# luk036/ellalgo-rs

Hardware: AMD Instinct MI355X
Metric: ellipsoid updates/sec at n=16384; achieved HBM GB/s vs peak (higher is better)
Workload: dtype f64

## Files before the change

ellalgo-rs_amd/capi.py:

```python
from __future__ import annotations

import ctypes as C
import os

from . import build as _build

SUCCESS, NOSOLN, NOEFFECT, UNKNOWN = 0, 1, 2, 3
CUT_BIAS, CUT_CENTRAL, CUT_Q = 0, 1, 2
SPACE_ELL, SPACE_ELL_STABLE = 0, 1
E_NORCCL = -6
SHARD_EQUAL_BLOCKS, SHARD_SYMMETRIC = 0, 1
NCCL_ID_BYTES = 128
E_INVALID, E_HIP, E_NODEVICE, E_NOMEM, E_STATE = -1, -2, -3, -4, -5
NKERNEL_CLASSES = 14
(OPT_AUTO_DEFER, OPT_SYMV, OPT_SYMV_MIN_N, OPT_APPLY_LOWER, OPT_APPLY_KERNEL, OPT_FUSE_DOTS, OPT_STABLE_SOLVE,
 OPT_STABLE_FACTOR, OPT_PAD, OPT_LP_GRID, OPT_LP_WIDE, OPT_BATCH_THREADS, OPT_RESIDENT, OPT_OVERLAP,
 OPT_LOOKAHEAD, OPT_QUEUE_DEPTH, OPT_RESIDENT_FAULT, OPT_RESIDENT_ABANDONED, OPT_STABLE_MIRRORED, OPT_STAGE_DIRECT) = range(1, 21)
KERNEL_CLASS_NAMES = ("gemv", "scalar", "rank1", "stable_fwd", "stable_bwd", "stable_factor", "fused", "apply",
                      "apply_gemv", "symv", "symv_reduce", "lp_scan", "lp_final", "resident")

EXPORTS = [
    "ellhip_create", "ellhip_create_shard", "ellhip_clone", "ellhip_destroy", "ellhip_update", "ellhip_tsq",
    "ellhip_get_xc", "ellhip_set_xc", "ellhip_kappa", "ellhip_ndim", "ellhip_get_mq",
    "ellhip_set_no_defer_trick", "ellhip_set_use_parallel_cut", "ellhip_set_defer_depth", "ellhip_defer_depth", "ellhip_flush", "ellhip_queue_primed", "ellhip_set_shard_symmetric", "ellhip_calc", "ellhip_update_begin",
    "ellhip_update_end", "ellhip_gt_dev", "ellhip_set_gt_dev", "ellhip_prime", "ellhip_cut", "ellhip_commit",
    "ellhip_queue_upload", "ellhip_queue_run", "ellhip_queue_run_fused", "ellhip_queue_begin", "ellhip_queue_end",
    "ellhip_queue_prime", "ellhip_queue_cut", "ellhip_queue_commit", "ellhip_queue_results", "ellhip_set_stream",
    "ellhip_synchronize", "ellhip_profile_enable", "ellhip_profile_read", "ellhip_device_count",
    "ellhip_last_error", "ellhip_version",
    "ellhip_set_option", "ellhip_get_option", "ellhip_set_default_option", "ellhip_default_option",
    "ellhip_lowpass_create", "ellhip_lowpass_destroy", "ellhip_lowpass_assess_feas", "ellhip_lowpass_assess_optim",
    "ellhip_lowpass_state", "ellhip_lowpass_rows_visited", "ellhip_lowpass_get_spectrum", "ellhip_lowpass_optim", "ellhip_lowpass_feas",
# ... 240 lines not shown
```

ellalgo-rs_amd/csrc/ell_kernels.hpp:

```cpp
#pragma once

#include <hip/hip_runtime.h>

#include "ellcalc_device.hpp"

namespace ellhip {

struct CutParams {
    int kind;
    int has_b1;
    double b0;
    double b1;
};

struct DevState {
    double kappa;
    double tsq;
    double omega;
    double ratio;
    double rho_over_omega;
    double scale;
    int status;
    int apply;
    int halted;
// ... 1068 lines not shown
    __shared__ double sgr[SYMV_H][SMM_NV2 + 1];
    __shared__ int s_t;
    if (st->halted) return;
    Q -= row0 * ld;
    for (;;) {
        __syncthreads();
        if (threadIdx.x == 0) {
            const unsigned t = atomicAdd(queue, 1u);
            s_t = t < (unsigned)ntiles ? (int)t : -1;
        }
        __syncthreads();
        const int t = s_t;
        if (t < 0) return;
        symm_tile2<NT, SEG>(Q, ld, n, row0, (long long)tiles[t].I, (long long)tiles[t].J, gT, lv, rowpart, colpart, rowpart_stride,
                            colpart_stride, sh, sgr);
    }
}

constexpr int PUB_WGS = 16;
__global__ __launch_bounds__(256) void k_publish(const DevState* __restrict__ st, const double* __restrict__ xc, long long n,
                                                 LiveMirror* __restrict__ m, double* __restrict__ h_xc,
                                                 unsigned long long seq, unsigned* __restrict__ arrived) {
    __shared__ int last;
    const long long n2 = n / 2;
    for (long long i = (long long)blockIdx.x * 256 + threadIdx.x; i < n2; i += (long long)gridDim.x * 256)
        *reinterpret_cast<double2_t*>(h_xc + 2 * i) = *reinterpret_cast<const double2_t*>(xc + 2 * i);
    if ((n & 1) && blockIdx.x == 0 && threadIdx.x == 0) h_xc[n - 1] = xc[n - 1];
    __threadfence_system();
    __syncthreads();
    if (threadIdx.x == 0) {
// ... 530 lines not shown
```

ellalgo-rs_amd/csrc/ellhip_capi.hip:

```cpp
#include "../../include/ellhip.h"

#include <hip/hip_runtime.h>

#include <cstddef>
#include <cstdio>
#include <cstdlib>
#include <algorithm>
#include <atomic>
#include <cstring>
#include <memory>
#include <mutex>
#include <new>
#include <string>
#include <vector>

#include "ell_kernels.hpp"
#include "ellstable_kernels.hpp"
#include "resident_kernels.hpp"
#include "group_kernels.hpp"

using namespace ellhip;

namespace {

// ... 24 lines not shown
    hipEvent_t a, b;
    int cls;
};

struct Defaults {
    int auto_defer = 1;
    int symv = 1;
    long long symv_min_n = 5120;
    int apply_lower = 1;
    int apply_kernel = -1;
    int fuse_dots = 1;
    int resident = 1;
    int overlap = 1;
    int lookahead = 32;
    int queue_depth = 48;
    int stable_solve = 3;
    int stable_factor = 2;
    int pad = -1;
    int lp_grid = 0;
    int lp_wide = -1;
    int batch_threads = 0;
    int stage_direct = 1;
};
Defaults g_defaults;

enum : int { CLS_GEMV = 0, CLS_SCALAR = 1, CLS_RANK1 = 2, CLS_ST_FWD = 3, CLS_ST_BWD = 4, CLS_ST_FACTOR = 5, CLS_FUSED = 6, CLS_APPLY = 7, CLS_APPLY_GEMV = 8, CLS_SYMV = 9, CLS_SYMV_REDUCE = 10, CLS_LP_SCAN = 11, CLS_LP_FINAL = 12, CLS_RESIDENT = 13 };

struct Shape {
    int rw = 0, unr = 0, nt = 0;
};
// ... 28 lines not shown
    int st_since_enter = 0;
    bool st_prev_persist = true;
    bool st_prev_helped = true;
    double* d_partial = nullptr;
    double* d_pend = nullptr;
    double* d_cpend = nullptr;
    double* d_rowpart = nullptr;
    double* d_colpart = nullptr;
    int overlap = 1;
    double* d_rowpart2 = nullptr;
    double* d_colpart2 = nullptr;
    int part_set = 0;
    hipStream_t symv_stream = nullptr;
    int lookahead = 32;
    int queue_depth = 48;
    double* d_rowpart_m = nullptr;
    double* d_colpart_m = nullptr;
    double* d_gT = nullptr;
    SymmTile* d_symm_tiles = nullptr;
    unsigned* d_symm_queue = nullptr;
    int symm_ntiles = 0, symm_wgs = 0;
    double* d_grpY = nullptr;
    double* d_gpart = nullptr;
    double* d_cpart = nullptr;
    double* d_gsums = nullptr;
    GroupOut* d_gout = nullptr;
    int (*grp_exchange)(void* ctx, double* buf, long long count, hipStream_t stream) = nullptr;
    void* grp_exchange_ctx = nullptr;
    hipEvent_t ev_symv = nullptr;
    hipEvent_t ev_side_go = nullptr;
// ... 139 lines not shown
        s->sh_fused = {4, 4, 0};
    } else {
        s->sh_gemv = {4, 4, 1};
        s->sh_rank1 = {2, 8, 1};
        s->sh_fused = {2, 8, 1};
    }
    s->sh_apply = {4, 1, s->sh_fused.nt};
    s->symv = g_defaults.symv;
    s->symv_min_n = g_defaults.symv_min_n;
    s->apply_lower = g_defaults.apply_lower;
    s->apply_kernel = g_defaults.apply_kernel;
    s->fuse_dots = g_defaults.fuse_dots;
    s->overlap = g_defaults.overlap;
    s->lookahead = g_defaults.lookahead;
    s->queue_depth = g_defaults.queue_depth;
    s->resident = g_defaults.resident;
    s->stable_solve = g_defaults.stable_solve;
    s->stable_factor = g_defaults.stable_factor;
}

template <int VEC, bool NT, bool R1, bool GV, bool SCALE>
int launch_sweep_t(ellhip_space* s, const Shape& sh, const double* gt_r1, const double* gvec, double* gv_out) {
    const long long nr = s->nrows;
    const unsigned grid = (unsigned)((nr + sh.rw - 1) / sh.rw);
    double* out = gv_out ? gv_out + s->row0 : nullptr;
#define SWEEP_CASE(RW, UNR)                                                                                  \
    if (sh.rw == RW && sh.unr == UNR) {                                                                      \
        hipLaunchKernelGGL((k_sweep<RW, UNR, VEC, NT, R1, GV, SCALE>), dim3(grid), dim3(256), 0, s->stream,  \
                           (const double*)s->d_Q, s->d_Q, s->ld, s->n, nr, s->row0, gt_r1, gvec, out, s->d_st, \
                           s->dir);                                                                          \
// ... 72 lines not shown
#define APPLY_CASE(RW, UNR)                                                                                   \
    if (sh.rw == RW && sh.unr == UNR) {                                                                       \
        hipLaunchKernelGGL((k_sweep_apply<RW, UNR, VEC, NT, GV, LOWER>), dim3(grid), dim3(256), 0, s->stream, \
                           (const double*)s->d_Q, s->d_Q, s->ld, s->n, nr, s->row0, (const double*)s->d_pend, \
                           (const double*)s->d_cpend, gvec, out, s->d_st, dir);                               \
        return 0;                                                                                             \
    }
    APPLY_CASE(1, 2) APPLY_CASE(1, 4) APPLY_CASE(2, 1) APPLY_CASE(2, 2) APPLY_CASE(2, 4) APPLY_CASE(4, 1) APPLY_CASE(4, 2)
#undef APPLY_CASE
    return fail(ELLHIP_E_INVALID, "unsupported ELLHIP_APPLY_RW/UNR shape (supported: 1x2 1x4 2x1 2x2 2x4 4x1 4x2)");
}

bool symv_ok(const ellhip_space* s);

int side_join(ellhip_space* s);
int flush_pending(ellhip_space* s, const double* gvec, double* gv_out) {
    {
        int jrc = side_join(s);
        if (jrc) return jrc;
        ProfScope ps(s, gvec ? CLS_APPLY_GEMV : CLS_APPLY);
        const bool even = (s->n % 2) == 0;
        const bool nt = even && s->sh_apply.nt;
        int rc;
        if (!gvec && s->apply_lower && symv_ok(s)) {
            const unsigned grid = (unsigned)((s->nrows + APL_TR - 1) / APL_TR);
#define APL_GO(NPV, NTV)                                                                                        \
    hipLaunchKernelGGL((k_apply_lower<NPV, NTV>), dim3(grid), dim3(256), 0, s->stream, s->d_Q, s->ld, s->n, s->nrows, \
                       s->row0, (const double*)s->d_pend, (const double*)s->d_cpend, (const DevState*)s->d_st)
            const bool deep = s->npend > s->defer;
            const int apply_kernel = deep ? 2 : (s->apply_kernel < 0 ? (s->defer == 24 ? 2 : 1) : s->apply_kernel);
// ... 22 lines not shown
            rc = 0;
            s->upper_stale = true;
        } else if (s->defer != 8) {
            return fail(ELLHIP_E_STATE, "defer depth 16 / 24 needs the lower-triangle schedule");
        } else if (gvec)
            rc = !even ? launch_apply_t<1, false, true>(s, gvec, gv_out)
                       : (nt ? launch_apply_t<2, true, true>(s, gvec, gv_out) : launch_apply_t<2, false, true>(s, gvec, gv_out));
        else
            rc = !even ? launch_apply_t<1, false, false>(s, nullptr, nullptr)
                       : (nt ? launch_apply_t<2, true, false>(s, nullptr, nullptr)
                             : launch_apply_t<2, false, false>(s, nullptr, nullptr));
        if (rc) return rc;
        HIPCHK(hipGetLastError());
        s->dir ^= 1;
    }
    hipLaunchKernelGGL(k_pend_reset, dim3(64), dim3(256), 0, s->stream, s->d_pend, s->d_cpend,
                       (long long)(s->npend > s->defer ? MAXPEND : s->defer) * s->n, s->d_st);
    HIPCHK(hipGetLastError());
    s->npend = 0;
    return 0;
}

int launch_mirror_if_needed(ellhip_space* s) {
    if (!s->needs_mirror) return 0;
    const unsigned t = (unsigned)((s->n + 31) / 32);
    hipLaunchKernelGGL(k_mirror_lower, dim3(t, t), dim3(256), 0, s->stream, s->d_Q, s->ld, s->n, s->d_st);
    HIPCHK(hipGetLastError());
    return 0;
}

constexpr int ST_MIRROR_PERIOD = 256;
int stable_mirror_enter(ellhip_space* s) {
    const unsigned t = (unsigned)((s->n + 63) / 64);
    hipLaunchKernelGGL(k_st_mirror_enter, dim3(t, t), dim3(256), 0, s->stream, s->d_Q, s->ld, s->n, (const DevState*)s->d_st,
                       s->d_rbuf);
// ... 967 lines not shown
                       (long long)colpart_elems(s), (const DevState*)s->d_st, (const SymmTile*)s->d_symm_tiles, 0, s->d_symm_queue)
        if (wide && nt) {
            ELLHIP_SYMM_WARM(k_symm_mfma_q<true, SYMV_SEG>);
            ELLHIP_SYMM_WARM(k_symm_mfma_q2<true, SYMV_SEG>);
        } else if (wide) {
            ELLHIP_SYMM_WARM(k_symm_mfma_q<false, SYMV_SEG>);
            ELLHIP_SYMM_WARM(k_symm_mfma_q2<false, SYMV_SEG>);
        } else if (nt) {
            ELLHIP_SYMM_WARM(k_symm_mfma_q<true, SYMV_SEG_SMALL>);
            ELLHIP_SYMM_WARM(k_symm_mfma_q2<true, SYMV_SEG_SMALL>);
        } else {
            ELLHIP_SYMM_WARM(k_symm_mfma_q<false, SYMV_SEG_SMALL>);
            ELLHIP_SYMM_WARM(k_symm_mfma_q2<false, SYMV_SEG_SMALL>);
        }
#undef ELLHIP_SYMM_WARM
        HIPCHK(hipGetLastError());
    }
    return 0;
}

template <int NP>
int group_stage_go(ellhip_space* s, long long i, int g, int half, int phase) {
    const unsigned nb = (unsigned)((s->n + 127) / 128);
    const double* grads = qgrad(s, i);
    if (phase == 0) {
        ProfScope ps(s, CLS_SYMV_REDUCE);
        const double* rowp = s->d_rowpart_m + (size_t)half * MULTI_MAX * rowpart_elems(s);
        const double* colp = s->d_colpart_m + (size_t)half * MULTI_MAX * colpart_elems(s);
        if (s->sharded)
            hipLaunchKernelGGL(k_group_reduce<0>, dim3(nb, (unsigned)g), dim3(256), 0, s->stream, s->n, s->row0, s->nrows,
// ... 40 lines not shown
    hipLaunchKernelGGL(k_pack_grads, dim3((unsigned)((s->n * nvw + 255) / 256)), dim3(256), 0, st, g_dev, s->n, lv, s->n, gT, queue, nvw);
    const bool nt = s->sh_gemv.nt != 0;
#define ELLHIP_SYMM_Q(...)                                                                                                          \
    hipLaunchKernelGGL((__VA_ARGS__), dim3((unsigned)wgs), dim3(256), 0, st, (const double*)s->d_Q, s->ld, s->n, s->row0,                \
                       (const double*)gT, lv, rowp, colp, (long long)rowpart_elems(s), (long long)colpart_elems(s),                 \
                       (const DevState*)s->d_st, (const SymmTile*)s->d_symm_tiles, s->symm_ntiles, queue)
    if (nvw == SMM_NV) {
        if (nt) ELLHIP_SYMM_Q(k_symm_mfma_q<true, SEG>);
        else ELLHIP_SYMM_Q(k_symm_mfma_q<false, SEG>);
    } else {
        if (nt) ELLHIP_SYMM_Q(k_symm_mfma_q2<true, SEG>);
        else ELLHIP_SYMM_Q(k_symm_mfma_q2<false, SEG>);
    }
#undef ELLHIP_SYMM_Q
}
long long group_size(const ellhip_space* s, long long cap, long long rem) {
    long long g = std::min(cap, rem);
    if (multi_mfma(s) && cap <= SMM_NV && rem > cap && rem < 2 * cap) g = (rem + 1) / 2;
    return g;
}

int symm_go(ellhip_space* s, const double* g_dev, int lv, hipStream_t st, int half, bool beside = false) {
    ProfScope ps(s, CLS_SYMV, st);
    const int wgs = beside ? std::max(1, s->symm_wgs - std::max(1, s->symm_wgs / 16)) : s->symm_wgs;
    if (s->symv_seg == SYMV_SEG) symm_mfma_go<SYMV_SEG>(s, g_dev, lv, st, half, wgs);
    else symm_mfma_go<SYMV_SEG_SMALL>(s, g_dev, lv, st, half, wgs);
    HIPCHK(hipGetLastError());
    return 0;
}

// ... 15 lines not shown
    int rc = multi_setup(s);
    if (rc) return rc;
    const long long end = first + count;
    if (s->sharded && (s->primed || !s->grp_exchange))
        return fail(ELLHIP_E_STATE, "group run of a row shard: the owner takes a primed cut by itself and supplies the collective");
    const bool deep_ok = multi_mfma(s) && s->defer == 24 && s->apply_lower && s->queue_depth > s->defer;
    const int qdepth = deep_ok ? s->queue_depth : s->defer;
    if (qdepth != 8 && qdepth != 16 && qdepth != 24 && qdepth != MAXPEND)
        return fail(ELLHIP_E_STATE, "queue run: recorded-update depth must be 8, 16, 24 or 48");
    const bool use_side = multi_mfma(s) && s->overlap != 0 && !s->sharded;
    if (use_side) {
        rc = side_setup(s);
        if (rc) return rc;
    }
    SideGuard guard{s};
    int half = 0;
    long long ahead_i = -1, ahead_g = 0;
    long long i = first;
    while (i < end) {
        long long g = 1;
        if (!(s->primed && s->primed_qindex == i)) {
            rc = ensure_committed(s);
            if (rc) return rc;
            const long long room = (long long)qdepth - s->npend;
            const long long cap = std::min<long long>(s->lookahead, multi_mfma(s) ? MULTI_MAX : MULTI_VALU_MAX);
            const long long rem = std::min(end - i, room);
            g = group_size(s, cap, rem);
        }
        if (g <= 1 && !s->sharded) {
            if (s->npend >= s->defer) {
                rc = flush_pending(s, nullptr, nullptr);
                if (rc) return rc;
            }
            rc = queue_prime_impl(s, i);
            if (!rc) rc = queue_cut_impl(s, i);
            if (!rc) rc = queue_commit_impl(s, i, -1);
            if (rc) return rc;
            i += 1;
            continue;
        }
        if (multi_mfma(s)) {
            const long long cap = MULTI_MAX;
            rc = side_join(s);
            if (rc) return rc;
            if (!(ahead_i == i && ahead_g == g)) {
                rc = symm_go(s, qgrad(s, i), (int)g, s->stream, half);
                if (rc) return rc;
            }
            ahead_i = -1;
            const long long i2 = i + g, room2 = (long long)qdepth - (s->npend + g);
            long long g2 = 0;
            if (i2 < end && room2 > 0) {
                const long long cap2 = std::min<long long>(s->lookahead, cap), rem2 = std::min(end - i2, room2);
                g2 = group_size(s, cap2, rem2);
            }
            drop_prime(s);
            s->dots_np = 0;
            s->xc_host_valid = false;
#define ELLHIP_STAGE(PHASE)                                                                                          \
    (qdepth == MAXPEND ? group_stage_go<MAXPEND>(s, i, (int)g, half, PHASE)                                          \
// ... 4 lines not shown
            if (use_side && g2 >= 2) {
                rc = side_fork(s);
                if (!rc) rc = symm_go(s, qgrad(s, i2), (int)g2, side_stream(s), half ^ 1, true);
                if (!rc) rc = side_mark(s);
                if (rc) return rc;
                ahead_i = i2;
                ahead_g = g2;
            }
            rc = ELLHIP_STAGE(1);
#undef ELLHIP_STAGE
            if (rc) return rc;
            s->npend += (int)g;
            s->scalars_stale = true;
            s->shrink_pending = false;
            if (s->npend >= qdepth) {
                rc = flush_pending(s, nullptr, nullptr);
                if (rc) return rc;
            }
            if (ahead_i >= 0) half ^= 1;
            i += g;
            continue;
        }
        {
            ProfScope ps(s, CLS_SYMV);
            const bool wide = s->symv_seg == SYMV_SEG;
            if (g == 2) {
                if (wide) symv_multi_go<SYMV_SEG, 2>(s, qgrad(s, i));
                else symv_multi_go<SYMV_SEG_SMALL, 2>(s, qgrad(s, i));
            } else {
                if (wide) symv_multi_go<SYMV_SEG, 3>(s, qgrad(s, i));
                else symv_multi_go<SYMV_SEG_SMALL, 3>(s, qgrad(s, i));
            }
// ... 249 lines not shown
    s->kappa = src->kappa;
    s->tsq = src->tsq;
    s->sh_gemv = src->sh_gemv;
    s->sh_rank1 = src->sh_rank1;
    s->sh_fused = src->sh_fused;
    s->sh_apply = src->sh_apply;
    s->symv = src->symv;
    s->symv_rw = src->symv_rw;
    s->symv_min_n = src->symv_min_n;
    s->apply_lower = src->apply_lower;
    s->apply_kernel = src->apply_kernel;
    s->fuse_dots = src->fuse_dots;
    s->overlap = src->overlap;
    s->lookahead = src->lookahead;
    s->queue_depth = src->queue_depth;
    s->resident = src->resident;
    s->shard_symmetric = src->shard_symmetric;
    s->upper_stale = src->upper_stale;
    s->symv_seg = src->symv_seg;
    s->stable_solve = src->stable_solve;
    s->stable_factor = src->stable_factor;
    rc = alloc_common(s);
    if (rc) {
        ellhip_destroy(s);
        return rc;
    }
    hipError_t e = hipStreamSynchronize(src->stream);
    if (e == hipSuccess)
        e = hipMemcpyAsync(s->d_Q, src->d_Q, (size_t)s->nrows * (size_t)s->ld * sizeof(double),
                           hipMemcpyDeviceToDevice, s->stream);
// ... 262 lines not shown
        return fail(ELLHIP_E_STATE, "symmetric row shard: set the mode before the first update");
    DeviceGuard guard(s->device);
    s->shard_symmetric = flag != 0;
    if (s->shard_symmetric && s->defer > 1) {
        int rc = symv_alloc(s);
        if (rc) return rc;
    }
    return 0;
}

namespace {
int option_ok(int key, long long v) {
    switch (key) {
        case ELLHIP_OPT_APPLY_KERNEL:
            return (v >= -1 && v <= 2) ? 0 : fail(ELLHIP_E_INVALID, "option value must be -1, 0, 1 or 2");
        case ELLHIP_OPT_STAGE_DIRECT: return (v == 0 || v == 1) ? 0 : fail(ELLHIP_E_INVALID, "option value must be 0 or 1");
        case ELLHIP_OPT_AUTO_DEFER: case ELLHIP_OPT_SYMV: case ELLHIP_OPT_APPLY_LOWER:
        case ELLHIP_OPT_FUSE_DOTS:
            return (v == 0 || v == 1) ? 0 : fail(ELLHIP_E_INVALID, "option value must be 0 or 1");
        case ELLHIP_OPT_RESIDENT: return (v >= 0 && v <= 2) ? 0 : fail(ELLHIP_E_INVALID, "ELLHIP_OPT_RESIDENT: 0, 1 or 2");
        case ELLHIP_OPT_OVERLAP: return (v >= 0 && v <= 2) ? 0 : fail(ELLHIP_E_INVALID, "ELLHIP_OPT_OVERLAP: 0, 1 or 2");
        case ELLHIP_OPT_LOOKAHEAD: return (v >= 1 && v <= 32) ? 0 : fail(ELLHIP_E_INVALID, "ELLHIP_OPT_LOOKAHEAD: 1 .. 32");
        case ELLHIP_OPT_QUEUE_DEPTH: return (v == 0 || v == 48) ? 0 : fail(ELLHIP_E_INVALID, "ELLHIP_OPT_QUEUE_DEPTH: 0 or 48");
        case ELLHIP_OPT_RESIDENT_FAULT: return v >= -1 ? 0 : fail(ELLHIP_E_INVALID, "ELLHIP_OPT_RESIDENT_FAULT: -1 or a cut index");
        case ELLHIP_OPT_SYMV_MIN_N: return v >= 512 ? 0 : fail(ELLHIP_E_INVALID, "ELLHIP_OPT_SYMV_MIN_N must be >= 512");
        case ELLHIP_OPT_STABLE_SOLVE: return (v >= 0 && v <= 3) ? 0 : fail(ELLHIP_E_INVALID, "ELLHIP_OPT_STABLE_SOLVE: 0 .. 3");
        case ELLHIP_OPT_STABLE_FACTOR:
            return (v >= 0 && v <= 2) ? 0 : fail(ELLHIP_E_INVALID, "option value must be 0, 1 or 2");
        case ELLHIP_OPT_PAD: return (v >= -1 && v <= 4096) ? 0 : fail(ELLHIP_E_INVALID, "ELLHIP_OPT_PAD: -1 .. 4096");
        case ELLHIP_OPT_LP_GRID: return (v >= 0 && v <= 65536) ? 0 : fail(ELLHIP_E_INVALID, "ELLHIP_OPT_LP_GRID: 0 .. 65536");
        case ELLHIP_OPT_LP_WIDE: return (v >= -1 && v <= 1) ? 0 : fail(ELLHIP_E_INVALID, "ELLHIP_OPT_LP_WIDE: -1, 0, 1");
// ... 6 lines not shown

int ellhip_set_default_option(int key, int64_t value) {
    int rc = option_ok(key, value);
    if (rc) return rc;
    switch (key) {
        case ELLHIP_OPT_AUTO_DEFER: g_defaults.auto_defer = (int)value; break;
        case ELLHIP_OPT_SYMV: g_defaults.symv = (int)value; break;
        case ELLHIP_OPT_SYMV_MIN_N: g_defaults.symv_min_n = value; break;
        case ELLHIP_OPT_APPLY_LOWER: g_defaults.apply_lower = (int)value; break;
        case ELLHIP_OPT_APPLY_KERNEL: g_defaults.apply_kernel = (int)value; break;
        case ELLHIP_OPT_FUSE_DOTS: g_defaults.fuse_dots = (int)value; break;
        case ELLHIP_OPT_RESIDENT: g_defaults.resident = (int)value; break;
        case ELLHIP_OPT_OVERLAP: g_defaults.overlap = (int)value; break;
        case ELLHIP_OPT_LOOKAHEAD: g_defaults.lookahead = (int)value; break;
        case ELLHIP_OPT_QUEUE_DEPTH: g_defaults.queue_depth = (int)value; break;
        case ELLHIP_OPT_STABLE_SOLVE: g_defaults.stable_solve = (int)value; break;
        case ELLHIP_OPT_STABLE_FACTOR: g_defaults.stable_factor = (int)value; break;
        case ELLHIP_OPT_PAD: g_defaults.pad = (int)value; break;
        case ELLHIP_OPT_LP_GRID: g_defaults.lp_grid = (int)value; break;
        case ELLHIP_OPT_LP_WIDE: g_defaults.lp_wide = (int)value; break;
        case ELLHIP_OPT_BATCH_THREADS: g_defaults.batch_threads = (int)value; break;
        case ELLHIP_OPT_STAGE_DIRECT: g_defaults.stage_direct = (int)value; break;
    }
    return 0;
}

int ellhip_default_option(int key, int64_t* value) {
    if (!value) return fail(ELLHIP_E_INVALID, "value is NULL");
    switch (key) {
        case ELLHIP_OPT_AUTO_DEFER: *value = g_defaults.auto_defer; break;
        case ELLHIP_OPT_SYMV: *value = g_defaults.symv; break;
        case ELLHIP_OPT_SYMV_MIN_N: *value = g_defaults.symv_min_n; break;
        case ELLHIP_OPT_APPLY_LOWER: *value = g_defaults.apply_lower; break;
        case ELLHIP_OPT_APPLY_KERNEL: *value = g_defaults.apply_kernel; break;
        case ELLHIP_OPT_FUSE_DOTS: *value = g_defaults.fuse_dots; break;
        case ELLHIP_OPT_RESIDENT: *value = g_defaults.resident; break;
        case ELLHIP_OPT_OVERLAP: *value = g_defaults.overlap; break;
        case ELLHIP_OPT_LOOKAHEAD: *value = g_defaults.lookahead; break;
        case ELLHIP_OPT_QUEUE_DEPTH: *value = g_defaults.queue_depth; break;
        case ELLHIP_OPT_STABLE_SOLVE: *value = g_defaults.stable_solve; break;
        case ELLHIP_OPT_STABLE_FACTOR: *value = g_defaults.stable_factor; break;
        case ELLHIP_OPT_PAD: *value = g_defaults.pad; break;
        case ELLHIP_OPT_LP_GRID: *value = g_defaults.lp_grid; break;
        case ELLHIP_OPT_LP_WIDE: *value = g_defaults.lp_wide; break;
        case ELLHIP_OPT_BATCH_THREADS: *value = g_defaults.batch_threads; break;
        case ELLHIP_OPT_STAGE_DIRECT: *value = g_defaults.stage_direct; break;
        default: return fail(ELLHIP_E_INVALID, "unknown option key");
    }
    return 0;
}

int ellhip_set_option(ellhip_space* s, int key, int64_t value) {
    if (!s) return fail(ELLHIP_E_INVALID, "NULL handle");
    int rc = option_ok(key, value);
// ... 4 lines not shown
        case ELLHIP_OPT_RESIDENT:
            if (!ell) return fail(ELLHIP_E_INVALID, "this option exists on Ell only");
            s->resident = (int)value;
            return 0;
        case ELLHIP_OPT_OVERLAP:
            if (!ell) return fail(ELLHIP_E_INVALID, "this option exists on Ell only");
            s->overlap = (int)value;
            return 0;
        case ELLHIP_OPT_LOOKAHEAD:
            if (!ell) return fail(ELLHIP_E_INVALID, "this option exists on Ell only");
            s->lookahead = (int)value;
            return 0;
        case ELLHIP_OPT_QUEUE_DEPTH:
            if (!ell) return fail(ELLHIP_E_INVALID, "this option exists on Ell only");
            s->queue_depth = (int)value;
            return 0;
        case ELLHIP_OPT_RESIDENT_FAULT:
            if (!ell) return fail(ELLHIP_E_INVALID, "this option exists on Ell only");
            s->rs_fault_at = value;
            return 0;
        case ELLHIP_OPT_SYMV: case ELLHIP_OPT_SYMV_MIN_N: case ELLHIP_OPT_APPLY_LOWER: case ELLHIP_OPT_APPLY_KERNEL:
        case ELLHIP_OPT_FUSE_DOTS: {
            if (!ell) return fail(ELLHIP_E_INVALID, "this option exists on Ell only");
            if (s->in_two_phase) return fail(ELLHIP_E_STATE, "update_begin without update_end");
            rc = make_q_current(s);
            if (rc) return rc;
            if (key == ELLHIP_OPT_SYMV) s->symv = (int)value;
            else if (key == ELLHIP_OPT_SYMV_MIN_N) s->symv_min_n = value;
            else if (key == ELLHIP_OPT_APPLY_LOWER) s->apply_lower = (int)value;
            else if (key == ELLHIP_OPT_APPLY_KERNEL) s->apply_kernel = (int)value;
// ... 21 lines not shown
    }
}

int ellhip_get_option(const ellhip_space* s, int key, int64_t* value) {
    if (!s || !value) return fail(ELLHIP_E_INVALID, "NULL argument");
    switch (key) {
        case ELLHIP_OPT_SYMV: *value = s->symv; break;
        case ELLHIP_OPT_SYMV_MIN_N: *value = s->symv_min_n; break;
        case ELLHIP_OPT_APPLY_LOWER: *value = s->apply_lower; break;
        case ELLHIP_OPT_APPLY_KERNEL: *value = s->apply_kernel; break;
        case ELLHIP_OPT_FUSE_DOTS: *value = s->fuse_dots; break;
        case ELLHIP_OPT_RESIDENT: *value = s->resident; break;
        case ELLHIP_OPT_OVERLAP: *value = s->overlap; break;
        case ELLHIP_OPT_LOOKAHEAD: *value = s->lookahead; break;
        case ELLHIP_OPT_QUEUE_DEPTH: *value = s->queue_depth; break;
        case ELLHIP_OPT_RESIDENT_FAULT: *value = s->rs_fault_at; break;
        case ELLHIP_OPT_RESIDENT_ABANDONED: *value = s->rs_abandoned; break;
        case ELLHIP_OPT_STABLE_SOLVE: *value = s->stable_solve; break;
        case ELLHIP_OPT_STABLE_FACTOR: *value = s->stable_factor; break;
        case ELLHIP_OPT_STABLE_MIRRORED: *value = s->st_mirrored ? 1 : 0; break;
        case ELLHIP_OPT_STAGE_DIRECT: *value = s->stage_direct ? 1 : 0; break;
        case ELLHIP_OPT_PAD: *value = s->ld - s->n; break;
        default: return fail(ELLHIP_E_INVALID, "not a per-handle option");
    }
    return 0;
}

int ellhip_set_use_parallel_cut(ellhip_space* s, int flag) {
    if (!s) return fail(ELLHIP_E_INVALID, "NULL handle");
    s->use_parallel_cut = flag ? 1 : 0;
// ... 212 lines not shown
```

include/ellhip.h:

```cpp
#ifndef ELLHIP_H
#define ELLHIP_H

#include <stdint.h>

#ifdef __cplusplus
extern "C" {
#endif

#define ELLHIP_SUCCESS 0
#define ELLHIP_NOSOLN 1
#define ELLHIP_NOEFFECT 2
#define ELLHIP_UNKNOWN 3

#define ELLHIP_E_INVALID (-1)
#define ELLHIP_E_HIP (-2)
#define ELLHIP_E_NODEVICE (-3)
#define ELLHIP_E_NOMEM (-4)
#define ELLHIP_E_STATE (-5)

#define ELLHIP_CUT_BIAS 0
#define ELLHIP_CUT_CENTRAL 1
#define ELLHIP_CUT_Q 2

#define ELLHIP_SPACE_ELL 0
// ... 50 lines not shown
#define ELLHIP_OPT_FUSE_DOTS 6
#define ELLHIP_OPT_STABLE_SOLVE 7
#define ELLHIP_OPT_STABLE_FACTOR 8
#define ELLHIP_OPT_PAD 9
#define ELLHIP_OPT_LP_GRID 10
#define ELLHIP_OPT_LP_WIDE 11
#define ELLHIP_OPT_BATCH_THREADS 12
#define ELLHIP_OPT_RESIDENT 13
#define ELLHIP_OPT_OVERLAP 14
#define ELLHIP_OPT_LOOKAHEAD 15
#define ELLHIP_OPT_QUEUE_DEPTH 16
#define ELLHIP_OPT_RESIDENT_FAULT 17
#define ELLHIP_OPT_RESIDENT_ABANDONED 18
#define ELLHIP_OPT_STABLE_MIRRORED 19
#define ELLHIP_OPT_STAGE_DIRECT 20
int ellhip_set_option(ellhip_space *s, int key, int64_t value);
int ellhip_get_option(const ellhip_space *s, int key, int64_t *value);
int ellhip_set_default_option(int key, int64_t value);
int ellhip_default_option(int key, int64_t *value);

int ellhip_queue_upload(ellhip_space *s, int64_t k, const int32_t *kinds, const double *grads,
                        const double *beta0, const int32_t *has_beta1, const double *beta1);
int ellhip_queue_run(ellhip_space *s, int64_t first, int64_t count);
int ellhip_queue_run_fused(ellhip_space *s, int64_t first, int64_t count);
int ellhip_queue_begin(ellhip_space *s, int64_t index);
int ellhip_queue_end(ellhip_space *s, int64_t index);
int ellhip_queue_prime(ellhip_space *s, int64_t index);
int ellhip_queue_cut(ellhip_space *s, int64_t index);
int ellhip_queue_commit(ellhip_space *s, int64_t index, int64_t next_index);
int ellhip_queue_results(ellhip_space *s, int32_t *status_out, double *tsq_out);
// ... 16 lines not shown
```

Baseline: 30940.

## Fuse deferred rank-k apply with next group's symmetric mat-mult pass over Q

Adds a kernel that applies the pending deferred low-rank updates to each lower-triangle tile of Q with f64 MFMA and, in the same pass, computes the symmetric product of the updated tile with the next group of gradients. The queue runner now marks the flush as owed and fuses it into the next group's symv instead of doing a separate apply sweep followed by a separate read of Q. This is meant to cut one full read/write pass over the n×n matrix per flush in a bandwidth-bound workload. It adds an option (on by default), more template instantiations, extra LDS use, and a guard that flushes if the loop exits while still owed.

Measured after the change: 34650, median of 6. 12.0% higher.

```diff
diff --git a/ellalgo-rs_amd/capi.py b/ellalgo-rs_amd/capi.py
--- a/ellalgo-rs_amd/capi.py
+++ b/ellalgo-rs_amd/capi.py
@@ -15,7 +15,8 @@
 NKERNEL_CLASSES = 14
 (OPT_AUTO_DEFER, OPT_SYMV, OPT_SYMV_MIN_N, OPT_APPLY_LOWER, OPT_APPLY_KERNEL, OPT_FUSE_DOTS, OPT_STABLE_SOLVE,
  OPT_STABLE_FACTOR, OPT_PAD, OPT_LP_GRID, OPT_LP_WIDE, OPT_BATCH_THREADS, OPT_RESIDENT, OPT_OVERLAP,
- OPT_LOOKAHEAD, OPT_QUEUE_DEPTH, OPT_RESIDENT_FAULT, OPT_RESIDENT_ABANDONED, OPT_STABLE_MIRRORED, OPT_STAGE_DIRECT) = range(1, 21)
+ OPT_LOOKAHEAD, OPT_QUEUE_DEPTH, OPT_RESIDENT_FAULT, OPT_RESIDENT_ABANDONED, OPT_STABLE_MIRRORED, OPT_STAGE_DIRECT,
+ OPT_APPLY_SYMM) = range(1, 22)
 KERNEL_CLASS_NAMES = ("gemv", "scalar", "rank1", "stable_fwd", "stable_bwd", "stable_factor", "fused", "apply",
                       "apply_gemv", "symv", "symv_reduce", "lp_scan", "lp_final", "resident")
 
diff --git a/ellalgo-rs_amd/csrc/ell_kernels.hpp b/ellalgo-rs_amd/csrc/ell_kernels.hpp
--- a/ellalgo-rs_amd/csrc/ell_kernels.hpp
+++ b/ellalgo-rs_amd/csrc/ell_kernels.hpp
@@ -1106,6 +1106,166 @@
         if (t < 0) return;
         symm_tile2<NT, SEG>(Q, ld, n, row0, (long long)tiles[t].I, (long long)tiles[t].J, gT, lv, rowpart, colpart, rowpart_stride,
                             colpart_stride, sh, sgr);
+    }
+}
+
+template <int NP, bool NT, int SEG, bool WIDE>
+__device__ __forceinline__ void apply_symm_tile(double* __restrict__ Q, long long ld, long long n, long long I, long long J,
+                                                const double* __restrict__ pend, const double* __restrict__ cpend,
+                                                const double* __restrict__ gT, int lv, double* __restrict__ rowpart,
+                                                double* __restrict__ colpart, long long rowpart_stride, long long colpart_stride,
+                                                bool prod, double (*sh)[SYMV_H * SMM_PITCH], double (*sgr)[SMM_NV2 + 1],
+                                                double* __restrict__ sa) {
+    constexpr int KS = NP / 4;
+    constexpr int NVT = WIDE ? 2 : 1;
+    constexpr int NVW = SMM_NV * NVT;
+    const int lane = threadIdx.x & 63, wave = threadIdx.x >> 6;
+    const int lr = lane >> 4, lc = lane & 15;
+    const long long r0 = I * SYMV_H;
+    const long long c0 = J * SEG;
+    const bool full = c0 + SEG - 1 < r0;
+    for (int e = threadIdx.x; e < 4 * KS * 64; e += 256) {
+        const int q = e / (KS * 64), s = (e / 64) % KS, ln = e % 64;
+        const int k = 4 * s + (ln >> 4);
+        sa[((q * (KS / 2) + s / 2) * 64 + ln) * 2 + (s & 1)] = -(cpend[k] * pend[(long long)k * n + r0 + 16 * q + (ln & 15)]);
+    }
+    if (prod)
+        for (int k = threadIdx.x; k < SYMV_H * NVW; k += 256) sgr[k / NVW][k % NVW] = gT[(r0 + k / NVW) * NVW + k % NVW];
+    __syncthreads();
+    double4_t dr[NVT][4];
+#pragma unroll
+    for (int t = 0; t < NVT; ++t)
+#pragma unroll
+        for (int jj = 0; jj < 4; ++jj) dr[t][jj] = double4_t{0.0, 0.0, 0.0, 0.0};
+    const long long cend = (c0 + SEG < r0 + SYMV_H) ? c0 + SEG : r0 + SYMV_H;
+    const int nblk = (int)((cend - c0) / 16);
+    double* mysh = sh[wave];
+    double* qbase = Q + (r0 + lr) * ld + lc;
+    const double* pbase = pend + (long long)lr * n + lc;
+    for (int b = wave; b < nblk; b += 4) {
+        const long long cb = c0 + 16 * (long long)b;
+        double x[16], bv[KS], gc[NVT][4];
+#pragma unroll
+        for (int j = 0; j < 16; ++j) x[j] = ld_stream<NT, double>(qbase + (long long)(4 * j) * ld + cb);
+#pragma unroll
+        for (int s = 0; s < KS; ++s) bv[s] = pbase[(long long)(4 * s) * n + cb];
+        __builtin_amdgcn_sched_barrier(0);
+        double4_t acc[4];
+#pragma unroll
+        for (int q = 0; q < 4; ++q) acc[q] = double4_t{x[4 * q], x[4 * q + 1], x[4 * q + 2], x[4 * q + 3]};
+#pragma unroll
+        for (int s2 = 0; s2 < KS / 2; ++s2)
+#pragma unroll
+            for (int q = 0; q < 4; ++q) {
+                const double2_t a = *reinterpret_cast<const double2_t*>(&sa[((q * (KS / 2) + s2) * 64 + lane) * 2]);
+                acc[q] = __builtin_amdgcn_mfma_f64_16x16x4f64(a.x, bv[2 * s2], acc[q], 0, 0, 0);
+                acc[q] = __builtin_amdgcn_mfma_f64_16x16x4f64(a.y, bv[2 * s2 + 1], acc[q], 0, 0, 0);
+                if (q == 3) __builtin_amdgcn_sched_barrier(0);
+            }
+#pragma unroll
+        for (int q = 0; q < 4; ++q) {
+            x[4 * q] = acc[q].x;
+            x[4 * q + 1] = acc[q].y;
+            x[4 * q + 2] = acc[q].z;
+            x[4 * q + 3] = acc[q].w;
+        }
+#pragma unroll
+        for (int j = 0; j < 16; ++j) qbase[(long long)(4 * j) * ld + cb] = x[j];
+        if (!prod) continue;
+        __builtin_amdgcn_sched_barrier(0);
+#pragma unroll
+        for (int t = 0; t < NVT; ++t)
+#pragma unroll
+            for (int kb = 0; kb < 4; ++kb) gc[t][kb] = gT[(cb + 4 * kb + lr) * NVW + 16 * t + lc];
+        const bool diag = !full && cb + 15 >= r0;
+        double4_t dc[NVT];
+#pragma unroll
+        for (int t = 0; t < NVT; ++t) {
+            dc[t] = double4_t{0.0, 0.0, 0.0, 0.0};
+#pragma unroll
+            for (int j = 0; j < 16; ++j) {
+                const long long r = r0 + 4 * j + lr, c = cb + lc;
+                const double below = (!diag || c < r) ? x[j] : 0.0;
+                dc[t] = __builtin_amdgcn_mfma_f64_16x16x4f64(sgr[4 * j + lr][16 * t + lc], below, dc[t], 0, 0, 0);
+            }
+        }
+        if (diag) {
+#pragma unroll
+            for (int j = 0; j < 16; ++j) {
+                const long long r = r0 + 4 * j + lr, c = cb + lc;
+                x[j] = (c <= r) ? x[j] : 0.0;
+            }
+        }
+#pragma unroll
+        for (int j = 0; j < 16; ++j) mysh[(4 * j + lr) * SMM_PITCH + lc] = x[j];
+#pragma unroll
+        for (int t = 0; t < NVT; ++t)
+#pragma unroll
+            for (int jj = 0; jj < 4; ++jj)
+#pragma unroll
+                for (int kb = 0; kb < 4; ++kb) {
+                    const double tv = mysh[(16 * jj + lc) * SMM_PITCH + 4 * kb + lr];
+                    dr[t][jj] = __builtin_amdgcn_mfma_f64_16x16x4f64(gc[t][kb], tv, dr[t][jj], 0, 0, 0);
+                }
+#pragma unroll
+        for (int t = 0; t < NVT; ++t) {
+            const double o[4] = {dc[t].x, dc[t].y, dc[t].z, dc[t].w};
+#pragma unroll
+            for (int i = 0; i < 4; ++i) {
+                const int v = 16 * t + lr + 4 * i;
+                if (v < lv) colpart[(long long)v * colpart_stride + I * n + cb + lc] = o[i];
+            }
+        }
+    }
+    if (!prod) return;
+    __syncthreads();
+    double* red = &sh[0][0];
+#pragma unroll
+    for (int t = 0; t < NVT; ++t) {
+#pragma unroll
+        for (int jj = 0; jj < 4; ++jj) {
+            const double o[4] = {dr[t][jj].x, dr[t][jj].y, dr[t][jj].z, dr[t][jj].w};
+#pragma unroll
+            for (int i = 0; i < 4; ++i) red[((wave * 4 + jj) * 4 + i) * 64 + lane] = o[i];
+        }
+        __syncthreads();
+#pragma unroll
+        for (int i = 0; i < 4; ++i) {
+            const int v = 16 * t + lr + 4 * i;
+            const int jj = wave;
+            const double s0 = red[((0 * 4 + jj) * 4 + i) * 64 + lane], s1 = red[((1 * 4 + jj) * 4 + i) * 64 + lane];
+            const double s2 = red[((2 * 4 + jj) * 4 + i) * 64 + lane], s3 = red[((3 * 4 + jj) * 4 + i) * 64 + lane];
+            if (v < lv) rowpart[(long long)v * rowpart_stride + J * n + r0 + 16 * jj + lc] = ((s0 + s1) + s2) + s3;
+        }
+        __syncthreads();
+    }
+}
+
+template <int NP, bool NT, int SEG, bool WIDE>
+__global__ __launch_bounds__(256, 2) void k_apply_symm_q(double* __restrict__ Q, long long ld, long long n,
+                                                         const double* __restrict__ pend, const double* __restrict__ cpend,
+                                                         const double* __restrict__ gT, int lv, double* __restrict__ rowpart,
+                                                         double* __restrict__ colpart, long long rowpart_stride,
+                                                         long long colpart_stride, const DevState* __restrict__ st,
+                                                         const SymmTile* __restrict__ tiles, int ntiles,
+                                                         unsigned* __restrict__ queue) {
+    static_assert(NP % 8 == 0, "k-steps taken in pairs");
+    __shared__ double sh[4][SYMV_H * SMM_PITCH];
+    __shared__ double sgr[SYMV_H][SMM_NV2 + 1];
+    __shared__ double sa[SYMV_H * NP];
+    __shared__ int s_t;
+    const bool prod = !st->halted;
+    for (;;) {
+        __syncthreads();
+        if (threadIdx.x == 0) {
+            const unsigned t = atomicAdd(queue, 1u);
+            s_t = t < (unsigned)ntiles ? (int)t : -1;
+        }
+        __syncthreads();
+        const int t = s_t;
+        if (t < 0) return;
+        apply_symm_tile<NP, NT, SEG, WIDE>(Q, ld, n, (long long)tiles[t].I, (long long)tiles[t].J, pend, cpend, gT, lv, rowpart,
+                                           colpart, rowpart_stride, colpart_stride, prod, sh, sgr, sa);
     }
 }
 
diff --git a/ellalgo-rs_amd/csrc/ellhip_capi.hip b/ellalgo-rs_amd/csrc/ellhip_capi.hip
--- a/ellalgo-rs_amd/csrc/ellhip_capi.hip
+++ b/ellalgo-rs_amd/csrc/ellhip_capi.hip
@@ -62,6 +62,7 @@
     int overlap = 1;
     int lookahead = 32;
     int queue_depth = 48;
+    int apply_symm = 1;
     int stable_solve = 3;
     int stable_factor = 2;
     int pad = -1;
@@ -120,6 +121,7 @@
     hipStream_t symv_stream = nullptr;
     int lookahead = 32;
     int queue_depth = 48;
+    int apply_symm = 1;
     double* d_rowpart_m = nullptr;
     double* d_colpart_m = nullptr;
     double* d_gT = nullptr;
@@ -289,6 +291,7 @@
     s->overlap = g_defaults.overlap;
     s->lookahead = g_defaults.lookahead;
     s->queue_depth = g_defaults.queue_depth;
+    s->apply_symm = g_defaults.apply_symm;
     s->resident = g_defaults.resident;
     s->stable_solve = g_defaults.stable_solve;
     s->stable_factor = g_defaults.stable_factor;
@@ -391,6 +394,13 @@
 bool symv_ok(const ellhip_space* s);
 
 int side_join(ellhip_space* s);
+int pend_reset(ellhip_space* s) {
+    hipLaunchKernelGGL(k_pend_reset, dim3(64), dim3(256), 0, s->stream, s->d_pend, s->d_cpend,
+                       (long long)(s->npend > s->defer ? MAXPEND : s->defer) * s->n, s->d_st);
+    HIPCHK(hipGetLastError());
+    s->npend = 0;
+    return 0;
+}
 int flush_pending(ellhip_space* s, const double* gvec, double* gv_out) {
     {
         int jrc = side_join(s);
@@ -443,11 +453,7 @@
         HIPCHK(hipGetLastError());
         s->dir ^= 1;
     }
-    hipLaunchKernelGGL(k_pend_reset, dim3(64), dim3(256), 0, s->stream, s->d_pend, s->d_cpend,
-                       (long long)(s->npend > s->defer ? MAXPEND : s->defer) * s->n, s->d_st);
-    HIPCHK(hipGetLastError());
-    s->npend = 0;
-    return 0;
+    return pend_reset(s);
 }
 
 int launch_mirror_if_needed(ellhip_space* s) {
@@ -1445,6 +1451,26 @@
             ELLHIP_SYMM_WARM(k_symm_mfma_q2<false, SYMV_SEG_SMALL>);
         }
 #undef ELLHIP_SYMM_WARM
+#define ELLHIP_APPLY_SYMM_WARM(...)                                                                                                  \
+    hipLaunchKernelGGL((__VA_ARGS__), dim3(1), dim3(256), 0, s->stream, s->d_Q, s->ld, s->n, (const double*)s->d_pend,               \
+                       (const double*)s->d_cpend, (const double*)s->d_gT, 0, s->d_rowpart_m, s->d_colpart_m,                         \
+                       (long long)rowpart_elems(s), (long long)colpart_elems(s), (const DevState*)s->d_st,                         \
+                       (const SymmTile*)s->d_symm_tiles, 0, s->d_symm_queue)
+#define ELLHIP_APPLY_SYMM_WARM4(NTV, SEGV)                         \
+    do {                                                           \
+        ELLHIP_APPLY_SYMM_WARM(k_apply_symm_q<MAXPEND, NTV, SEGV, true>);  \
+        ELLHIP_APPLY_SYMM_WARM(k_apply_symm_q<MAXPEND, NTV, SEGV, false>); \
+        ELLHIP_APPLY_SYMM_WARM(k_apply_symm_q<24, NTV, SEGV, true>);       \
+        ELLHIP_APPLY_SYMM_WARM(k_apply_symm_q<24, NTV, SEGV, false>);      \
+    } while (0)
+        if (s->row0 == 0 && !s->sharded) {
+            if (wide && nt) ELLHIP_APPLY_SYMM_WARM4(true, SYMV_SEG);
+            else if (wide) ELLHIP_APPLY_SYMM_WARM4(false, SYMV_SEG);
+            else if (nt) ELLHIP_APPLY_SYMM_WARM4(true, SYMV_SEG_SMALL);
+            else ELLHIP_APPLY_SYMM_WARM4(false, SYMV_SEG_SMALL);
+        }
+#undef ELLHIP_APPLY_SYMM_WARM4
+#undef ELLHIP_APPLY_SYMM_WARM
         HIPCHK(hipGetLastError());
     }
     return 0;
@@ -1515,6 +1541,68 @@
     }
 #undef ELLHIP_SYMM_Q
 }
+int apply_symm_np(const ellhip_space* s) {
+    if (!s->apply_symm || s->sharded || s->variant != ELLHIP_SPACE_ELL || !s->apply_lower || !symv_ok(s) || !multi_mfma(s) ||
+        s->symm_ntiles == 0)
+        return 0;
+    if (s->npend > s->defer) return MAXPEND;
+    const int apply_kernel = s->apply_kernel < 0 ? (s->defer == 24 ? 2 : 1) : s->apply_kernel;
+    return (apply_kernel == 2 && s->defer == 24) ? 24 : 0;
+}
+
+template <int SEG>
+void apply_symm_mfma_go(ellhip_space* s, const double* g_dev, int lv, int half, int np) {
+    double* gT = s->d_gT + (size_t)half * (size_t)s->n * MULTI_MAX;
+    double* rowp = s->d_rowpart_m + (size_t)half * MULTI_MAX * rowpart_elems(s);
+    double* colp = s->d_colpart_m + (size_t)half * MULTI_MAX * colpart_elems(s);
+    unsigned* queue = s->d_symm_queue + 32 * half;
+    const int nvw = lv > SMM_NV ? SMM_NV2 : SMM_NV;
+    hipLaunchKernelGGL(k_pack_grads, dim3((unsigned)((s->n * nvw + 255) / 256)), dim3(256), 0, s->stream, g_dev, s->n, lv, s->n, gT,
+                       queue, nvw);
+    const bool nt = s->sh_gemv.nt != 0;
+#define ELLHIP_APPLY_SYMM(...)                                                                                                      \
+    hipLaunchKernelGGL((__VA_ARGS__), dim3((unsigned)s->symm_wgs), dim3(256), 0, s->stream, s->d_Q, s->ld, s->n,                    \
+                       (const double*)s->d_pend, (const double*)s->d_cpend, (const double*)gT, lv, rowp, colp,                      \
+                       (long long)rowpart_elems(s), (long long)colpart_elems(s), (const DevState*)s->d_st,                         \
+                       (const SymmTile*)s->d_symm_tiles, s->symm_ntiles, queue)
+#define ELLHIP_APPLY_SYMM_NP(NPV)                                                                                                   \
+    if (nvw == SMM_NV) {                                                                                                            \
+        if (nt) ELLHIP_APPLY_SYMM(k_apply_symm_q<NPV, true, SEG, false>);                                                           \
+        else ELLHIP_APPLY_SYMM(k_apply_symm_q<NPV, false, SEG, false>);                                                             \
+    } else {                                                                                                                        \
+        if (nt) ELLHIP_APPLY_SYMM(k_apply_symm_q<NPV, true, SEG, true>);                                                            \
+        else ELLHIP_APPLY_SYMM(k_apply_symm_q<NPV, false, SEG, true>);                                                              \
+    }
+    if (np == MAXPEND) {
+        ELLHIP_APPLY_SYMM_NP(MAXPEND)
+    } else {
+        ELLHIP_APPLY_SYMM_NP(24)
+    }
+#undef ELLHIP_APPLY_SYMM_NP
+#undef ELLHIP_APPLY_SYMM
+}
+int apply_symm_go(ellhip_space* s, const double* g_dev, int lv, int half, int np, bool& owed) {
+    {
+        ProfScope ps(s, CLS_APPLY_GEMV);
+        if (s->symv_seg == SYMV_SEG) apply_symm_mfma_go<SYMV_SEG>(s, g_dev, lv, half, np);
+        else apply_symm_mfma_go<SYMV_SEG_SMALL>(s, g_dev, lv, half, np);
+        HIPCHK(hipGetLastError());
+    }
+    owed = false;
+    s->upper_stale = true;
+    s->dir ^= 1;
+    return pend_reset(s);
+}
+struct OwedGuard {
+    ellhip_space* s;
+    bool& owed;
+    ~OwedGuard() {
+        if (!owed) return;
+        owed = false;
+        (void)flush_pending(s, nullptr, nullptr);
+    }
+};
+
 long long group_size(const ellhip_space* s, long long cap, long long rem) {
     long long g = std::min(cap, rem);
     if (multi_mfma(s) && cap <= SMM_NV && rem > cap && rem < 2 * cap) g = (rem + 1) / 2;
@@ -1560,6 +1648,8 @@
         if (rc) return rc;
     }
     SideGuard guard{s};
+    bool owed = false;
+    OwedGuard oguard{s, owed};
     int half = 0;
     long long ahead_i = -1, ahead_g = 0;
     long long i = first;
@@ -1568,13 +1658,14 @@
         if (!(s->primed && s->primed_qindex == i)) {
             rc = ensure_committed(s);
             if (rc) return rc;
-            const long long room = (long long)qdepth - s->npend;
+            const long long room = (long long)qdepth - (owed ? 0 : s->npend);
             const long long cap = std::min<long long>(s->lookahead, multi_mfma(s) ? MULTI_MAX : MULTI_VALU_MAX);
             const long long rem = std::min(end - i, room);
             g = group_size(s, cap, rem);
         }
         if (g <= 1 && !s->sharded) {
             if (s->npend >= s->defer) {
+                owed = false;
                 rc = flush_pending(s, nullptr, nullptr);
                 if (rc) return rc;
             }
@@ -1589,7 +1680,10 @@
             const long long cap = MULTI_MAX;
             rc = side_join(s);
             if (rc) return rc;
-            if (!(ahead_i == i && ahead_g == g)) {
+            if (owed) {
+                rc = apply_symm_go(s, qgrad(s, i), (int)g, half, apply_symm_np(s), owed);
+                if (rc) return rc;
+            } else if (!(ahead_i == i && ahead_g == g)) {
                 rc = symm_go(s, qgrad(s, i), (int)g, s->stream, half);
                 if (rc) return rc;
             }
@@ -1624,8 +1718,16 @@
             s->scalars_stale = true;
             s->shrink_pending = false;
             if (s->npend >= qdepth) {
-                rc = flush_pending(s, nullptr, nullptr);
-                if (rc) return rc;
+                const long long in = i + g;
+                long long gn = 0;
+                if (in < end && apply_symm_np(s) != 0)
+                    gn = group_size(s, std::min<long long>(s->lookahead, MULTI_MAX), std::min<long long>(end - in, qdepth));
+                if (gn >= 2 && in + gn < end) {
+                    owed = true;
+                } else {
+                    rc = flush_pending(s, nullptr, nullptr);
+                    if (rc) return rc;
+                }
             }
             if (ahead_i >= 0) half ^= 1;
             i += g;
@@ -1905,6 +2007,7 @@
     s->overlap = src->overlap;
     s->lookahead = src->lookahead;
     s->queue_depth = src->queue_depth;
+    s->apply_symm = src->apply_symm;
     s->resident = src->resident;
     s->shard_symmetric = src->shard_symmetric;
     s->upper_stale = src->upper_stale;
@@ -2197,7 +2300,8 @@
     switch (key) {
         case ELLHIP_OPT_APPLY_KERNEL:
             return (v >= -1 && v <= 2) ? 0 : fail(ELLHIP_E_INVALID, "option value must be -1, 0, 1 or 2");
-        case ELLHIP_OPT_STAGE_DIRECT: return (v == 0 || v == 1) ? 0 : fail(ELLHIP_E_INVALID, "option value must be 0 or 1");
+        case ELLHIP_OPT_STAGE_DIRECT: case ELLHIP_OPT_APPLY_SYMM:
+            return (v == 0 || v == 1) ? 0 : fail(ELLHIP_E_INVALID, "option value must be 0 or 1");
         case ELLHIP_OPT_AUTO_DEFER: case ELLHIP_OPT_SYMV: case ELLHIP_OPT_APPLY_LOWER:
         case ELLHIP_OPT_FUSE_DOTS:
             return (v == 0 || v == 1) ? 0 : fail(ELLHIP_E_INVALID, "option value must be 0 or 1");
@@ -2234,6 +2338,7 @@
         case ELLHIP_OPT_OVERLAP: g_defaults.overlap = (int)value; break;
         case ELLHIP_OPT_LOOKAHEAD: g_defaults.lookahead = (int)value; break;
         case ELLHIP_OPT_QUEUE_DEPTH: g_defaults.queue_depth = (int)value; break;
+        case ELLHIP_OPT_APPLY_SYMM: g_defaults.apply_symm = (int)value; break;
         case ELLHIP_OPT_STABLE_SOLVE: g_defaults.stable_solve = (int)value; break;
         case ELLHIP_OPT_STABLE_FACTOR: g_defaults.stable_factor = (int)value; break;
         case ELLHIP_OPT_PAD: g_defaults.pad = (int)value; break;
@@ -2258,6 +2363,7 @@
         case ELLHIP_OPT_OVERLAP: *value = g_defaults.overlap; break;
         case ELLHIP_OPT_LOOKAHEAD: *value = g_defaults.lookahead; break;
         case ELLHIP_OPT_QUEUE_DEPTH: *value = g_defaults.queue_depth; break;
+        case ELLHIP_OPT_APPLY_SYMM: *value = g_defaults.apply_symm; break;
         case ELLHIP_OPT_STABLE_SOLVE: *value = g_defaults.stable_solve; break;
         case ELLHIP_OPT_STABLE_FACTOR: *value = g_defaults.stable_factor; break;
         case ELLHIP_OPT_PAD: *value = g_defaults.pad; break;
@@ -2292,6 +2398,10 @@
         case ELLHIP_OPT_QUEUE_DEPTH:
             if (!ell) return fail(ELLHIP_E_INVALID, "this option exists on Ell only");
             s->queue_depth = (int)value;
+            return 0;
+        case ELLHIP_OPT_APPLY_SYMM:
+            if (!ell) return fail(ELLHIP_E_INVALID, "this option exists on Ell only");
+            s->apply_symm = (int)value;
             return 0;
         case ELLHIP_OPT_RESIDENT_FAULT:
             if (!ell) return fail(ELLHIP_E_INVALID, "this option exists on Ell only");
@@ -2343,6 +2453,7 @@
         case ELLHIP_OPT_OVERLAP: *value = s->overlap; break;
         case ELLHIP_OPT_LOOKAHEAD: *value = s->lookahead; break;
         case ELLHIP_OPT_QUEUE_DEPTH: *value = s->queue_depth; break;
+        case ELLHIP_OPT_APPLY_SYMM: *value = s->apply_symm; break;
         case ELLHIP_OPT_RESIDENT_FAULT: *value = s->rs_fault_at; break;
         case ELLHIP_OPT_RESIDENT_ABANDONED: *value = s->rs_abandoned; break;
         case ELLHIP_OPT_STABLE_SOLVE: *value = s->stable_solve; break;
diff --git a/include/ellhip.h b/include/ellhip.h
--- a/include/ellhip.h
+++ b/include/ellhip.h
@@ -88,6 +88,7 @@
 #define ELLHIP_OPT_RESIDENT_ABANDONED 18
 #define ELLHIP_OPT_STABLE_MIRRORED 19
 #define ELLHIP_OPT_STAGE_DIRECT 20
+#define ELLHIP_OPT_APPLY_SYMM 21
 int ellhip_set_option(ellhip_space *s, int key, int64_t value);
 int ellhip_get_option(const ellhip_space *s, int key, int64_t *value);
 int ellhip_set_default_option(int key, int64_t value);
```
